# johanDDC/R-TuckER

Measured on AMD Instinct MI355X. Metric: 1-vs-N triples scored/sec, higher is better.
Workload: dtype f32

## Files before the change

r-tucker_amd/csrc/rtk_score_cg_kernel.h:

```cpp
#pragma once
#include "rtk_common.h"
#include "rtk_pack.h"
#include <type_traits>

namespace rtk_cg {

#ifdef RTK_CG_STAMPS
static __device__ unsigned long long g_cg_tl[256 * 2 * 64];
#define RTK_CG_TL(role, code)                                                                                   \
    do {                                                                                                        \
        if (tl_on && tl_n < 64) {                                                                               \
            g_cg_tl[(blockIdx.x * 2 + (role)) * 64 + tl_n] =                                                    \
                ((unsigned long long)(code) << 56) | (__builtin_amdgcn_s_memtime() & 0x00ffffffffffffffull);    \
            ++tl_n;                                                                                             \
        }                                                                                                       \
    } while (0)
#define RTK_CG_TLR(role, code)                                                                                  \
    do {                                                                                                        \
        if (tl_on && tl_n < 64) {                                                                               \
            g_cg_tl[(blockIdx.x * 2 + (role)) * 64 + tl_n] =                                                    \
                ((unsigned long long)(code) << 56) | (__builtin_amdgcn_s_memrealtime() & 0x00ffffffffffffffull); \
            ++tl_n;                                                                                             \
        }                                                                                                       \
    } while (0)
#else
#define RTK_CG_TL(role, code) do { (void)tl_on; (void)tl_n; } while (0)
#define RTK_CG_TLR(role, code) do { (void)tl_on; (void)tl_n; } while (0)
#endif

constexpr int NG = 5;
constexpr int EX_BYTES = 4 * 4 * 64 * 16;
constexpr int MISC_BYTES = 1024;

template <int KS>
__host__ __device__ constexpr int tile_bytes() { return RTK_PACK_HDR + 2 * KS * 1024; }

template <int KS>
inline size_t lds_bytes(int) { return MISC_BYTES + 2 * (size_t)tile_bytes<KS>() + 4 * (size_t)EX_BYTES; }

__host__ __device__ constexpr int s_begin(int KS, int w) { return (KS * w + 3) / 4; }
__host__ __device__ constexpr int s_end(int KS, int w) { return (KS * (w + 1) + 3) / 4; }

struct Geo {
    int B, N, c, U, n_mt;
    int gq, gr;
    int64_t ld_out;
    __device__ __forceinline__ int first_group(int u) const {
        if (U <= 32768) return gq * u + (int)((unsigned)(gr * u) / (unsigned)U);
        return (int)((((int64_t)gq * U + gr) * u) / U);
    }
    __device__ __forceinline__ void set(int u, int &gb, int &n_g) const {
        gb = first_group(u);
        n_g = first_group(u + 1) - gb;
    }
};

typedef float f32x2 __attribute__((ext_vector_type(2)));
typedef _Float16 f16x2 __attribute__((ext_vector_type(2)));

__device__ __forceinline__ void split8(const f32x4 a, const f32x4 b, float up, f16x8 &hi, f16x8 &lo) {
    const f32x2 u2 = {up, up};
    f32x2 y[4] = {{a[0], a[1]}, {a[2], a[3]}, {b[0], b[1]}, {b[2], b[3]}};
    union { f16x2 h2[4]; f16x8 h8; unsigned u[4]; } H, Lo;
#pragma unroll
    for (int j = 0; j < 4; ++j) {
        y[j] = y[j] * u2;
        H.h2[j] = __builtin_convertvector(y[j], f16x2);
        unsigned l;
        asm("v_fma_mixlo_f16 %0, %1, 1.0, -%2 op_sel_hi:[0,0,1]" : "=v"(l) : "v"(y[j][0]), "v"(H.u[j]));
        asm("v_fma_mixhi_f16 %0, %1, 1.0, -%2 op_sel:[0,0,1] op_sel_hi:[0,0,1]" : "+v"(l) : "v"(y[j][1]), "v"(H.u[j]));
        Lo.u[j] = l;
    }
    hi = H.h8;
    lo = Lo.h8;
}

template <int KS, int K0, int K1>
__device__ __forceinline__ void load_fragments_raw(__amdgpu_buffer_rsrc_t rs, unsigned n_bytes, int row, int c, int h, f32x4 *rw) {
    const unsigned base = (unsigned)(row * c + 8 * h) * 4u;
    const int k_last = 16 * (KS - 1) + 8 * h;
    const unsigned base_a = (k_last + 4 <= c) ? base : n_bytes, base_b = (k_last + 8 <= c) ? base : n_bytes;
#pragma unroll
    for (int ks = K0; ks < K1; ++ks) {
        const bool last = ks + 1 == KS;
        rw[2 * (ks - K0)] = __builtin_bit_cast(f32x4, __builtin_amdgcn_raw_buffer_load_b128(rs, last ? base_a : base, 64 * ks, 0));
        rw[2 * (ks - K0) + 1] = __builtin_bit_cast(f32x4, __builtin_amdgcn_raw_buffer_load_b128(rs, last ? base_b : base, 64 * ks + 16, 0));
    }
}

template <int NP>
__device__ __forceinline__ float row_absmax(const f32x4 *rw) {
    float mx = 0.f;
#pragma unroll
    for (int i = 0; i + 1 < NP; i += 2) {
#pragma unroll
        for (int q = 0; q < 4; ++q)
            asm("v_max3_f32 %0, |%1|, |%2|, %0" : "+v"(mx) : "v"(rw[i][q]), "v"(rw[i + 1][q]));
    }
    return fmaxf(mx, __shfl_xor(mx, 32));
}

struct LdsMap {
    unsigned char *hdr;
    float *uso5;
    float *pmax;
    unsigned char *stg0, *stg1;
    unsigned char *exo;
    unsigned char *exp5;
    template <int KS>
    __device__ __forceinline__ void init(unsigned char *lds) {
        hdr = lds;
        uso5 = reinterpret_cast<float *>(lds + 384);
        pmax = reinterpret_cast<float *>(lds + 512);
        stg0 = lds + MISC_BYTES;
        stg1 = stg0 + tile_bytes<KS>();
        exo = stg1 + tile_bytes<KS>();
        exp5 = exo + 2 * EX_BYTES;
    }
};

struct MOut {
    float *out;
    int64_t ld_out;
    int B, nts;
    unsigned voff;
};

template <int KS, int W4, int SIGMOID, bool EXTRA>
__device__ __forceinline__ void m_sweep(const LdsMap &L, int cnt, int lane, const f16x8 (&BF)[2 * KS],
                                        const f16x8 *SF, float us_o, const MOut &mo, bool tl_on, int &tl_n) {
#ifndef RTK_CG_PF
#define RTK_CG_PF 3
#endif
    constexpr int PF = KS < RTK_CG_PF ? KS : RTK_CG_PF;
    constexpr int S0 = s_begin(KS, W4), S1 = s_end(KS, W4), NS = EXTRA ? S1 - S0 : 0;
    constexpr int NGAP = 3 * KS + 3 * NS;
    constexpr int PW0 = !EXTRA ? (1 << 20) : (NS > 0 ? 3 * S1 + 3 * NS + 2 : 32);
    constexpr int GEND = EXTRA ? (PW0 + 4 > 36 ? PW0 + 4 : 36) : 32;
    constexpr bool MSIG = SIGMOID == 2;
    const int h = lane >> 5;
    const float kfac = MSIG ? us_o * -1.4426950408889634f : us_o;
    float ee = 0.f;
    f32x16 accA, accB, accS;
#pragma unroll
    for (int e = 0; e < 16; ++e) accB[e] = 0.f, accS[e] = 0.f;
    const f32x16 zero = {0.f, 0.f, 0.f, 0.f, 0.f, 0.f, 0.f, 0.f, 0.f, 0.f, 0.f, 0.f, 0.f, 0.f, 0.f, 0.f};

    auto iteration = [&](auto par_c, auto chain_c, auto pieces_c, int i, f32x16 &accC, f32x16 &accP) {
        constexpr int PAR = decltype(par_c)::value;
        constexpr bool chain = decltype(chain_c)::value, pieces = decltype(pieces_c)::value;
        constexpr bool direct = !chain && pieces;
        f32x4 *exw = reinterpret_cast<f32x4 *>(L.exo + (PAR ^ 1) * EX_BYTES + W4 * 4096);
        f32x4 *exs = reinterpret_cast<f32x4 *>(L.exp5 + PAR * EX_BYTES + W4 * 4096);
        const float *rfp = reinterpret_cast<const float *>(L.hdr + ((i + 2) % 3) * 128) + 4 * h;
        f32x4 rfq[2];
        auto gap = [&](int g) {
            if (EXTRA && g >= PW0 && g < PW0 + 4) {
                if (chain) {
                    const int q = g - PW0;
                    exs[q * 64 + lane] = f32x4{accS[4 * q], accS[4 * q + 1], accS[4 * q + 2], accS[4 * q + 3]};
                }
                return;
            }
            const int p = g - ((EXTRA && g >= PW0 + 4) ? 4 : 0);
            if (p >= 32 || !pieces) return;
            const int e = p >> 1, eg = e >> 2;
            if ((p & 7) == 1 && eg < 3) rfq[(eg + 1) & 1] = *reinterpret_cast<const f32x4 *>(rfp + 8 * (eg + 1));
            if (MSIG) {
                if (!(p & 1)) {
                    ee = __builtin_amdgcn_exp2f(accP[e] * rfq[eg & 1][e & 3] * kfac);
                } else {
                    accP[e] = __builtin_amdgcn_rcpf(1.0f + ee);
                    if ((e & 3) == 3 && !direct) exw[eg * 64 + lane] = f32x4{accP[e - 3], accP[e - 2], accP[e - 1], accP[e]};
                }
            } else if ((p & 7) == 0) {
                f32x4 z;
#pragma unroll
                for (int q = 0; q < 4; ++q) z[q] = accP[4 * eg + q] * rfq[eg & 1][q] * kfac;
                if (direct) {
#pragma unroll
                    for (int q = 0; q < 4; ++q) accP[4 * eg + q] = (SIGMOID == 1) ? rtk_sigmoid(z[q]) : z[q];
                } else {
                    exw[eg * 64 + lane] = z;
                }
            }
        };
        if (pieces) rfq[0] = *reinterpret_cast<const f32x4 *>(rfp);
        if constexpr (chain) {
            const unsigned char *tile = PAR ? L.stg1 : L.stg0;
            const f16x8 *lh = reinterpret_cast<const f16x8 *>(tile + RTK_PACK_HDR);
            const f16x8 *ll = lh + KS * 64;
            f16x8 fa[PF], fl[PF];
#pragma unroll
            for (int p = 0; p < PF; ++p) {
                fa[p] = lh[p * 64 + lane];
                fl[p] = ll[p * 64 + lane];
            }
            int g = 0;
#pragma unroll
            for (int ks = 0; ks < KS; ++ks) {
                const f16x8 ah = fa[ks % PF], al = fl[ks % PF];
                if (ks + PF < KS) {
                    fa[ks % PF] = lh[(ks + PF) * 64 + lane];
                    fl[ks % PF] = ll[(ks + PF) * 64 + lane];
                }
                const bool sh = EXTRA && ks >= S0 && ks < S1;
                __builtin_amdgcn_sched_barrier(0);
                accC = __builtin_amdgcn_mfma_f32_32x32x16_f16(ah, BF[2 * ks], ks == 0 ? zero : accC, 0, 0, 0);
                __builtin_amdgcn_sched_barrier(0);
                gap(g++);
                __builtin_amdgcn_sched_barrier(0);
                if (sh) {
                    accS = __builtin_amdgcn_mfma_f32_32x32x16_f16(ah, SF[2 * (ks - S0)], ks == S0 ? zero : accS, 0, 0, 0);
                    __builtin_amdgcn_sched_barrier(0);
                    gap(g++);
                    __builtin_amdgcn_sched_barrier(0);
                }
                accC = __builtin_amdgcn_mfma_f32_32x32x16_f16(ah, BF[2 * ks + 1], accC, 0, 0, 0);
                __builtin_amdgcn_sched_barrier(0);
                gap(g++);
                __builtin_amdgcn_sched_barrier(0);
                if (sh) {
                    accS = __builtin_amdgcn_mfma_f32_32x32x16_f16(ah, SF[2 * (ks - S0) + 1], accS, 0, 0, 0);
                    __builtin_amdgcn_sched_barrier(0);
                    gap(g++);
                    __builtin_amdgcn_sched_barrier(0);
                }
                accC = __builtin_amdgcn_mfma_f32_32x32x16_f16(al, BF[2 * ks], accC, 0, 0, 0);
                __builtin_amdgcn_sched_barrier(0);
                gap(g++);
                __builtin_amdgcn_sched_barrier(0);
                if (sh) {
                    accS = __builtin_amdgcn_mfma_f32_32x32x16_f16(al, SF[2 * (ks - S0)], accS, 0, 0, 0);
                    __builtin_amdgcn_sched_barrier(0);
                    gap(g++);
                    __builtin_amdgcn_sched_barrier(0);
                }
            }
#pragma unroll
            for (int gg = NGAP; gg < GEND; ++gg) gap(gg);
        } else if constexpr (pieces) {
#pragma unroll
            for (int gg = 0; gg < 32; ++gg) gap(gg + ((EXTRA && gg >= PW0) ? 4 : 0));
            const __amdgpu_buffer_rsrc_t rs = __builtin_amdgcn_make_buffer_rsrc(
                mo.out + (int64_t)(i - 1) * 32 * mo.ld_out, 0, (unsigned)(min(32, mo.B - (i - 1) * 32) * mo.ld_out * 4), 0x00020000);
            const unsigned ld4 = (unsigned)(mo.ld_out * 4);
            auto put = [&](auto aux_c) {
                unsigned off = mo.voff;
#pragma unroll
                for (int e = 0; e < 16; ++e) {
                    const float pe = accP[e];
                    __builtin_amdgcn_raw_buffer_store_b32(__builtin_bit_cast(unsigned, pe), rs, off, 0, decltype(aux_c)::value);
                    off += ((e & 3) == 3) ? 5u * ld4 : ld4;
                }
            };
            if (mo.nts) put(std::integral_constant<int, 2>{});
            else put(std::integral_constant<int, 0>{});
        }
        RTK_CG_TL(0, 6);
        __syncthreads();
        RTK_CG_TL(0, 5);
    };
    using P0 = std::integral_constant<int, 0>;
    using P1 = std::integral_constant<int, 1>;
    using T = std::true_type;
    using F = std::false_type;
    iteration(P0{}, T{}, F{}, 0, accA, accB);
    int i = 1;
    for (; i + 1 < cnt; i += 2) {
        iteration(P1{}, T{}, T{}, i, accB, accA);
        iteration(P0{}, T{}, T{}, i + 1, accA, accB);
    }
    if (i < cnt) {
        iteration(P1{}, T{}, T{}, i, accB, accA);
        iteration(P0{}, F{}, T{}, i + 1, accA, accB);
    } else {
        iteration(P1{}, F{}, T{}, i, accB, accA);
    }
}

template <int KS, int W4, int SIGMOID>
__device__ __forceinline__ void m_role(const Geo &geo, const float *__restrict__ O, float *__restrict__ out,
                                       const LdsMap &L, int lane, int nts) {
    constexpr int S0 = s_begin(KS, W4), S1 = s_end(KS, W4), NS = S1 - S0;
    const int r = lane & 31, h = lane >> 5, c = geo.c;
    const bool tl_on = W4 == 0 && lane == 0;
    int tl_n = 0;
    RTK_CG_TLR(0, 12);
    for (int u = blockIdx.x; u < geo.U; u += gridDim.x) {
        int gb, n_g;
        geo.set(u, gb, n_g);
        RTK_CG_TL(0, 1);
        const bool own = W4 < n_g;
        constexpr int NSX = NS > 0 ? NS : 1;
        f16x8 BF[2 * KS], SF[2 * NSX];
        float us_o = 0.f;
        {
            const int64_t row0 = (int64_t)gb * 32;
            const int valid_rows = (int)max((int64_t)0, min((int64_t)n_g * 32, (int64_t)geo.N - row0));
            const __amdgpu_buffer_rsrc_t rs = __builtin_amdgcn_make_buffer_rsrc(
                const_cast<float *>(O + row0 * c), 0, (unsigned)valid_rows * (unsigned)c * 4u, 0x00020000);
            const unsigned n_bytes = (unsigned)valid_rows * (unsigned)c * 4u;
            if (NS > 0) load_fragments_raw<KS, S0, S1>(rs, n_bytes, 4 * 32 + r, c, h, reinterpret_cast<f32x4 *>(SF));
            load_fragments_raw<KS, 0, KS>(rs, n_bytes, W4 * 32 + r, c, h, reinterpret_cast<f32x4 *>(BF));
            const float pm = NS > 0 ? row_absmax<2 * NSX>(reinterpret_cast<const f32x4 *>(SF)) : 0.f;
            if (h == 0) L.pmax[W4 * 32 + r] = pm;
            RTK_CG_TL(0, 2);
            __syncthreads();
            if (n_g == NG) {
                const float m5 = fmaxf(fmaxf(L.pmax[r], L.pmax[32 + r]), fmaxf(L.pmax[64 + r], L.pmax[96 + r]));
                const int sh5 = rtk_pack_shift(m5);
                const float up5 = ldexpf(1.0f, sh5);
#pragma unroll
                for (int ks = 0; ks < NS; ++ks)
                    split8(__builtin_bit_cast(f32x4, SF[2 * ks]), __builtin_bit_cast(f32x4, SF[2 * ks + 1]), up5, SF[2 * ks], SF[2 * ks + 1]);
                if (W4 == 0 && h == 0) L.uso5[r] = ldexpf(1.0f, -sh5);
            }
            RTK_CG_TL(0, 7);
            if (own) {
                const int sh = rtk_pack_shift(row_absmax<2 * KS>(reinterpret_cast<const f32x4 *>(BF)));
                const float up = ldexpf(1.0f, sh);
#pragma unroll
                for (int ks = 0; ks < KS; ++ks)
                    split8(__builtin_bit_cast(f32x4, BF[2 * ks]), __builtin_bit_cast(f32x4, BF[2 * ks + 1]), up, BF[2 * ks], BF[2 * ks + 1]);
                us_o = ldexpf(1.0f, -sh);
            }
        }
        RTK_CG_TL(0, 3);
        __syncthreads();
        RTK_CG_TL(0, 4);
        MOut mo;
        mo.out = out; mo.ld_out = geo.ld_out; mo.B = geo.B; mo.nts = nts;
        {
            const int j = (gb + W4) * 32 + r;
            mo.voff = (own && j < geo.N) ? (unsigned)(4 * h * geo.ld_out * 4) + (unsigned)j * 4u : 0x80000000u;
        }
        if (!own) {
            for (int i = 0; i < geo.n_mt + 1; ++i) __syncthreads();
        } else if (n_g == NG) {
            m_sweep<KS, W4, SIGMOID, true>(L, geo.n_mt, lane, BF, SF, us_o, mo, tl_on, tl_n);
        } else {
            m_sweep<KS, W4, SIGMOID, false>(L, geo.n_mt, lane, BF, SF, us_o, mo, tl_on, tl_n);
        }
    }
    RTK_CG_TLR(0, 13);
}

template <int AUX>
__device__ __forceinline__ void store_five(const float (&p5)[4], __amdgpu_buffer_rsrc_t rs, unsigned voff, unsigned ld4) {
    unsigned off = voff;
#pragma unroll
    for (int q = 0; q < 4; ++q) {
        __builtin_amdgcn_raw_buffer_store_b32(__builtin_bit_cast(unsigned, p5[q]), rs, off, 0, AUX);
        off += ld4;
    }
}

template <int KS>
__device__ __forceinline__ void h_prologue(const unsigned char *__restrict__ q_packed, const LdsMap &L, int t) {
    constexpr int TILE_BYTES = tile_bytes<KS>();
    constexpr int CHUNKS = TILE_BYTES / 16;
    constexpr int NLD = (CHUNKS + 255) / 256;
    const int ht = t & 255;
    u32x4 sreg[NLD];
    const u32x4 *src = reinterpret_cast<const u32x4 *>(q_packed);
#pragma unroll
    for (int i = 0; i < NLD; ++i) {
        const int ch = i * 256 + ht;
        if (i + 1 < NLD || ch < CHUNKS) sreg[i] = src[ch];
    }
    u32x4 *dst = reinterpret_cast<u32x4 *>(L.stg0);
#pragma unroll
    for (int i = 0; i < NLD; ++i) {
        const int ch = i * 256 + ht;
        if (i + 1 < NLD || ch < CHUNKS) dst[ch] = sreg[i];
    }
    if (ht < RTK_PACK_HDR / 16) reinterpret_cast<u32x4 *>(L.hdr)[ht] = sreg[0];
}

template <int KS, int SIGMOID, int SW>
__device__ __forceinline__ void s_role(const Geo &geo, const unsigned char *__restrict__ q_packed,
                                       float *__restrict__ out, const LdsMap &L, int lane, int t, int nts, int tune) {
    constexpr int NU = (20 - SW + 2) / 3;
    const int r = lane & 31, h = lane >> 5, N = geo.N, B = geo.B;
    const int64_t ld_out = geo.ld_out;
    const unsigned ld4 = (unsigned)(ld_out * 4);
    const int cnt = geo.n_mt;
    const bool tl_on = SW == 0 && lane == 0;
    int tl_n = 0;
    for (int u = blockIdx.x; u < geo.U; u += gridDim.x) {
        int gb, n_g;
        geo.set(u, gb, n_g);
        RTK_CG_TL(1, 1);
        h_prologue<KS>(q_packed, L, t);
        RTK_CG_TL(1, 2);
        const bool five = n_g == NG;
        __syncthreads();
        __syncthreads();
        RTK_CG_TL(1, 4);
        const unsigned row4h = (unsigned)(4 * h * ld_out * 4);
        unsigned colb[5];
#pragma unroll
        for (int g = 0; g < 5; ++g) {
            const int j = (gb + g) * 32 + r;
            colb[g] = (g < n_g && j < N) ? row4h + (unsigned)j * 4u : 0x80000000u;
        }
        float k5 = five ? L.uso5[r] : 0.f;
        if (SIGMOID == 2) k5 *= -1.4426950408889634f;
        for (int i = 0; i < cnt + 1; ++i) {
            const bool st_own = i >= 2, st5 = five && i >= 1 && i <= cnt;
            f32x4 z[NU], p1[2], p2[2], p3[2], rf[2];
            const f32x4 *ex = reinterpret_cast<const f32x4 *>(L.exo + (i & 1) * EX_BYTES) + lane;
            const f32x4 *pr = reinterpret_cast<const f32x4 *>(L.exp5 + ((i - 1) & 1) * EX_BYTES) + lane;
            const unsigned char *rp = L.hdr + ((i + 2) % 3) * 128 + 4 * h * 4;
#pragma unroll
            for (int k = 0; k < NU; ++k) {
                constexpr int dummy = 0;
                (void)dummy;
                const int uu = SW + 3 * k;
                if (uu < 16) {
                    if (st_own) z[k] = ex[(uu >> 2) * 256 + (uu & 3) * 64];
                } else if (st5) {
                    const int b = uu - 16, kk = k - (NU - (SW == 2 ? 1 : (SW == 1 ? 2 : 1)));
                    z[k] = pr[b * 64];
                    p1[kk] = pr[256 + b * 64];
                    p2[kk] = pr[512 + b * 64];
                    p3[kk] = pr[768 + b * 64];
                    rf[kk] = *reinterpret_cast<const f32x4 *>(rp + b * 32);
                }
            }
            RTK_CG_TL(1, 11);
            const __amdgpu_buffer_rsrc_t rs_own = __builtin_amdgcn_make_buffer_rsrc(
                out + (int64_t)(i - 2) * 32 * ld_out, 0, (unsigned)(min(32, B - (i - 2) * 32) * ld_out * 4), 0x00020000);
            const __amdgpu_buffer_rsrc_t rs5 = __builtin_amdgcn_make_buffer_rsrc(
                out + (int64_t)(i - 1) * 32 * ld_out, 0, (unsigned)(min(32, B - (i - 1) * 32) * ld_out * 4), 0x00020000);
#pragma unroll
            for (int k = 0; k < NU; ++k) {
                const int uu = SW + 3 * k;
                float p[4];
                if (uu < 16) {
                    if (!st_own) continue;
#pragma unroll
                    for (int q = 0; q < 4; ++q) p[q] = (SIGMOID == 1) ? rtk_sigmoid(z[k][q]) : z[k][q];
                    const unsigned voff = colb[uu >> 2] + (unsigned)(uu & 3) * 8u * ld4;
                    if (tune & 16) asm volatile("" ::"v"(p[0]), "v"(p[1]), "v"(p[2]), "v"(p[3]));
                    else if (nts) store_five<2>(p, rs_own, voff, ld4);
                    else store_five<0>(p, rs_own, voff, ld4);
                } else {
                    if (!st5) continue;
                    const int b = uu - 16, kk = k - (NU - (SW == 2 ? 1 : (SW == 1 ? 2 : 1)));
#pragma unroll
                    for (int q = 0; q < 4; ++q) {
                        const float zz = (((z[k][q] + p1[kk][q]) + p2[kk][q]) + p3[kk][q]) * rf[kk][q] * k5;
                        p[q] = SIGMOID == 2 ? __builtin_amdgcn_rcpf(1.0f + __builtin_amdgcn_exp2f(zz))
                                            : (SIGMOID == 1 ? rtk_sigmoid(zz) : zz);
                    }
                    const unsigned voff = colb[4] + (unsigned)b * 8u * ld4;
                    if (tune & 16) asm volatile("" ::"v"(p[0]), "v"(p[1]), "v"(p[2]), "v"(p[3]));
                    else if (nts) store_five<2>(p, rs5, voff, ld4);
                    else store_five<0>(p, rs5, voff, ld4);
                }
            }
            RTK_CG_TL(1, 6);
            __syncthreads();
            RTK_CG_TL(1, 5);
        }
    }
}

template <int KS>
__device__ __forceinline__ void l_role(const Geo &geo, const unsigned char *__restrict__ q_packed,
                                       const LdsMap &L, int lane, int t, int tune) {
    constexpr int TILE_BYTES = tile_bytes<KS>();
    constexpr int CHUNKS = TILE_BYTES / 16;
    constexpr int NLD = (CHUNKS + 63) / 64;
    const int cnt = geo.n_mt;
    u32x4 sreg[NLD];
    const __amdgpu_buffer_rsrc_t rsq = __builtin_amdgcn_make_buffer_rsrc(
        const_cast<unsigned char *>(q_packed), 0, (unsigned)(cnt * TILE_BYTES), 0x00020000);
    auto stage_load = [&](int mt) {
#pragma unroll
        for (int i = 0; i < NLD; ++i)
            sreg[i] = __builtin_amdgcn_raw_buffer_load_b128(rsq, (unsigned)lane * 16u, mt * TILE_BYTES + i * 1024, 0);
    };
    auto stage_store = [&](int mt) {
        u32x4 *dst = reinterpret_cast<u32x4 *>((mt & 1) ? L.stg1 : L.stg0);
#pragma unroll
        for (int i = 0; i < NLD; ++i) {
            const int ch = i * 64 + lane;
            if (i + 1 < NLD || ch < CHUNKS) dst[ch] = sreg[i];
        }
        if (lane < RTK_PACK_HDR / 16) reinterpret_cast<u32x4 *>(L.hdr + (mt % 3) * 128)[lane] = sreg[0];
    };
    for (int u = blockIdx.x; u < geo.U; u += gridDim.x) {
        int gb, n_g;
        geo.set(u, gb, n_g);
        h_prologue<KS>(q_packed, L, t);
        if (cnt > 1 && !(tune & 32)) stage_load(1);
        __syncthreads();
        __syncthreads();
        for (int i = 0; i < cnt + 1; ++i) {
            if (i + 1 < cnt && !(tune & 32)) stage_store(i + 1);
            if (i + 2 < cnt && !(tune & 32)) stage_load(i + 2);
            __syncthreads();
        }
    }
}

template <int KS, int SIGMOID>
__global__ __launch_bounds__(512, 2) void score_cg_kernel(
    const unsigned char *__restrict__ q_packed, int B, const float *__restrict__ O, int N, int c,
    float *__restrict__ out, int64_t ld_out, int U, int gq, int gr, int nts, int tune) {
    extern __shared__ __attribute__((aligned(16))) unsigned char lds[];
    LdsMap L;
    L.init<KS>(lds);
    const int t = threadIdx.x, lane = t & 63, wave = t >> 6;
    Geo geo;
    geo.B = B; geo.N = N; geo.c = c; geo.U = U; geo.gq = gq; geo.gr = gr; geo.n_mt = (B + 31) / 32; geo.ld_out = ld_out;
    const int uwave = __builtin_amdgcn_readfirstlane(wave);
    {
        const int pr = __builtin_amdgcn_readfirstlane(uwave >= 4 ? (tune & 3) : ((tune >> 2) & 3));
        if (pr == 1) __builtin_amdgcn_s_setprio(1);
        else if (pr == 2) __builtin_amdgcn_s_setprio(2);
        else if (pr == 3) __builtin_amdgcn_s_setprio(3);
    }
#ifdef RTK_CG_STAMPS
    if ((uwave == 0 || uwave == 4) && lane == 0)
        g_cg_tl[(blockIdx.x * 2 + (uwave >> 2)) * 64 + 63] = __builtin_amdgcn_s_memtime();
#endif
    if (uwave == 0) m_role<KS, 0, SIGMOID>(geo, O, out, L, lane, __builtin_amdgcn_readfirstlane(nts));
    else if (uwave == 1) m_role<KS, 1, SIGMOID>(geo, O, out, L, lane, __builtin_amdgcn_readfirstlane(nts));
    else if (uwave == 2) m_role<KS, 2, SIGMOID>(geo, O, out, L, lane, __builtin_amdgcn_readfirstlane(nts));
    else if (uwave == 3) m_role<KS, 3, SIGMOID>(geo, O, out, L, lane, __builtin_amdgcn_readfirstlane(nts));
    else if (uwave == 4) s_role<KS, SIGMOID, 0>(geo, q_packed, out, L, lane, t, __builtin_amdgcn_readfirstlane(nts), __builtin_amdgcn_readfirstlane(tune));
    else if (uwave == 5) s_role<KS, SIGMOID, 1>(geo, q_packed, out, L, lane, t, __builtin_amdgcn_readfirstlane(nts), __builtin_amdgcn_readfirstlane(tune));
    else if (uwave == 6) s_role<KS, SIGMOID, 2>(geo, q_packed, out, L, lane, t, __builtin_amdgcn_readfirstlane(nts), __builtin_amdgcn_readfirstlane(tune));
    else l_role<KS>(geo, q_packed, L, lane, t, __builtin_amdgcn_readfirstlane(tune));
}

}
```

Baseline: 11.42 million.

## Pipeline fp32-to-split-fp16 fragment conversion into the first tile's MFMA chain

The prologue used to split every owned and shared k-step fragment into hi/lo fp16 before the first barrier. Now it converts only the first k-step. The remaining conversions are done in three stages (scale, round/lo, hi) and slotted into the gap slots between MFMAs of tile 0's chain, so they overlap matrix work instead of stalling it. The row absmax is computed before the barrier, and the sweep tail loop is restructured. This raises register pressure and adds scheduling complexity, and the extra-group path now runs m_sweep even for non-owning waves.

New measurement: 11.37 million. Within noise of the previous version (-0.4%).

```diff
diff --git a/r-tucker_amd/csrc/rtk_score_cg_kernel.h b/r-tucker_amd/csrc/rtk_score_cg_kernel.h
--- a/r-tucker_amd/csrc/rtk_score_cg_kernel.h
+++ b/r-tucker_amd/csrc/rtk_score_cg_kernel.h
@@ -58,21 +58,35 @@
 typedef float f32x2 __attribute__((ext_vector_type(2)));
 typedef _Float16 f16x2 __attribute__((ext_vector_type(2)));
 
+struct Split {
+    f32x2 y[4];
+    unsigned h[4], l[4];
+    __device__ __forceinline__ void scale(const f32x4 a, const f32x4 b, f32x2 up2) {
+        const f32x2 r[4] = {{a[0], a[1]}, {a[2], a[3]}, {b[0], b[1]}, {b[2], b[3]}};
+#pragma unroll
+        for (int j = 0; j < 4; ++j) asm volatile("v_pk_mul_f32 %0, %1, %2" : "=v"(y[j]) : "v"(r[j]), "v"(up2));
+    }
+    __device__ __forceinline__ void round_lo() {
+#pragma unroll
+        for (int j = 0; j < 4; ++j) asm volatile("v_cvt_pk_f16_f32 %0, %1, %2" : "=v"(h[j]) : "v"(y[j][0]), "v"(y[j][1]));
+#pragma unroll
+        for (int j = 0; j < 4; ++j)
+            asm volatile("v_fma_mixlo_f16 %0, %1, 1.0, -%2 op_sel_hi:[0,0,1]" : "=v"(l[j]) : "v"(y[j][0]), "v"(h[j]));
+    }
+    __device__ __forceinline__ void hi_out(f16x8 &hi, f16x8 &lo) {
+#pragma unroll
+        for (int j = 0; j < 4; ++j)
+            asm volatile("v_fma_mixhi_f16 %0, %1, 1.0, -%2 op_sel:[0,0,1] op_sel_hi:[0,0,1]" : "+v"(l[j]) : "v"(y[j][1]), "v"(h[j]));
+        hi = __builtin_bit_cast(f16x8, u32x4{h[0], h[1], h[2], h[3]});
+        lo = __builtin_bit_cast(f16x8, u32x4{l[0], l[1], l[2], l[3]});
+    }
+};
+
 __device__ __forceinline__ void split8(const f32x4 a, const f32x4 b, float up, f16x8 &hi, f16x8 &lo) {
-    const f32x2 u2 = {up, up};
-    f32x2 y[4] = {{a[0], a[1]}, {a[2], a[3]}, {b[0], b[1]}, {b[2], b[3]}};
-    union { f16x2 h2[4]; f16x8 h8; unsigned u[4]; } H, Lo;
-#pragma unroll
-    for (int j = 0; j < 4; ++j) {
-        y[j] = y[j] * u2;
-        H.h2[j] = __builtin_convertvector(y[j], f16x2);
-        unsigned l;
-        asm("v_fma_mixlo_f16 %0, %1, 1.0, -%2 op_sel_hi:[0,0,1]" : "=v"(l) : "v"(y[j][0]), "v"(H.u[j]));
-        asm("v_fma_mixhi_f16 %0, %1, 1.0, -%2 op_sel:[0,0,1] op_sel_hi:[0,0,1]" : "+v"(l) : "v"(y[j][1]), "v"(H.u[j]));
-        Lo.u[j] = l;
-    }
-    hi = H.h8;
-    lo = Lo.h8;
+    Split sp;
+    sp.scale(a, b, f32x2{up, up});
+    sp.round_lo();
+    sp.hi_out(hi, lo);
 }
 
 template <int KS, int K0, int K1>
@@ -126,9 +140,15 @@
     unsigned voff;
 };
 
-template <int KS, int W4, int SIGMOID, bool EXTRA>
-__device__ __forceinline__ void m_sweep(const LdsMap &L, int cnt, int lane, const f16x8 (&BF)[2 * KS],
-                                        const f16x8 *SF, float us_o, const MOut &mo, bool tl_on, int &tl_n) {
+#ifdef RTK_CG_SERIAL_PROLOGUE
+constexpr bool PIPELINED = false;
+#else
+constexpr bool PIPELINED = true;
+#endif
+
+template <int KS, int W4, int SIGMOID, bool EXTRA, int NSX>
+__device__ __forceinline__ void m_sweep(const LdsMap &L, int cnt, int lane, f16x8 (&BF)[2 * KS], f16x8 (&SF)[2 * NSX],
+                                        float up, float up5, float us_o, const MOut &mo, bool tl_on, int &tl_n) {
 #ifndef RTK_CG_PF
 #define RTK_CG_PF 3
 #endif
@@ -140,16 +160,19 @@
     constexpr bool MSIG = SIGMOID == 2;
     const int h = lane >> 5;
     const float kfac = MSIG ? us_o * -1.4426950408889634f : us_o;
+    const f32x2 up2 = {up, up}, up52 = {up5, up5};
     float ee = 0.f;
     f32x16 accA, accB, accS;
 #pragma unroll
     for (int e = 0; e < 16; ++e) accB[e] = 0.f, accS[e] = 0.f;
     const f32x16 zero = {0.f, 0.f, 0.f, 0.f, 0.f, 0.f, 0.f, 0.f, 0.f, 0.f, 0.f, 0.f, 0.f, 0.f, 0.f, 0.f};
 
-    auto iteration = [&](auto par_c, auto chain_c, auto pieces_c, int i, f32x16 &accC, f32x16 &accP) {
+    auto iteration = [&](auto par_c, auto chain_c, auto pieces_c, auto convert_c, int i, f32x16 &accC, f32x16 &accP) {
         constexpr int PAR = decltype(par_c)::value;
         constexpr bool chain = decltype(chain_c)::value, pieces = decltype(pieces_c)::value;
+        constexpr bool convert = decltype(convert_c)::value && PIPELINED;
         constexpr bool direct = !chain && pieces;
+        static_assert(!convert || (chain && !pieces), "the conversion rides in tile 0's chain");
         f32x4 *exw = reinterpret_cast<f32x4 *>(L.exo + (PAR ^ 1) * EX_BYTES + W4 * 4096);
         f32x4 *exs = reinterpret_cast<f32x4 *>(L.exp5 + PAR * EX_BYTES + W4 * 4096);
         const float *rfp = reinterpret_cast<const float *>(L.hdr + ((i + 2) % 3) * 128) + 4 * h;
@@ -185,6 +208,19 @@
                 }
             }
         };
+        Split cs[2];
+        auto stage = [&](auto which_c, int kk, int st) {
+            constexpr int X = decltype(which_c)::value;
+            f16x8 &fh = X ? SF[2 * kk] : BF[2 * kk], &fl = X ? SF[2 * kk + 1] : BF[2 * kk + 1];
+            if (st == 0) cs[X].scale(__builtin_bit_cast(f32x4, fh), __builtin_bit_cast(f32x4, fl), X ? up52 : up2);
+            else if (st == 1) cs[X].round_lo();
+            else cs[X].hi_out(fh, fl);
+        };
+        auto convert_ahead = [&](int ks, int slot, int nslots) {
+            const bool own_next = ks + 1 < KS, sh_next = EXTRA && ks + 1 >= S0 && ks + 1 < S1;
+            if (own_next && slot < 3) stage(std::integral_constant<int, 0>{}, ks + 1, slot);
+            if (sh_next && slot >= nslots - 3) stage(std::integral_constant<int, 1>{}, ks + 1 - S0, slot - (nslots - 3));
+        };
         if (pieces) rfq[0] = *reinterpret_cast<const f32x4 *>(rfp);
         if constexpr (chain) {
             const unsigned char *tile = PAR ? L.stg1 : L.stg0;
@@ -205,38 +241,46 @@
                     fl[ks % PF] = ll[(ks + PF) * 64 + lane];
                 }
                 const bool sh = EXTRA && ks >= S0 && ks < S1;
+                int slot = 0;
+                auto fill = [&] {
+                    gap(g++);
+                    if constexpr (convert) convert_ahead(ks, slot, sh ? 6 : 3);
+                    ++slot;
+                };
+                if (convert && ks == 0) RTK_CG_TL(0, 14);
                 __builtin_amdgcn_sched_barrier(0);
                 accC = __builtin_amdgcn_mfma_f32_32x32x16_f16(ah, BF[2 * ks], ks == 0 ? zero : accC, 0, 0, 0);
                 __builtin_amdgcn_sched_barrier(0);
-                gap(g++);
+                fill();
                 __builtin_amdgcn_sched_barrier(0);
                 if (sh) {
                     accS = __builtin_amdgcn_mfma_f32_32x32x16_f16(ah, SF[2 * (ks - S0)], ks == S0 ? zero : accS, 0, 0, 0);
                     __builtin_amdgcn_sched_barrier(0);
-                    gap(g++);
+                    fill();
                     __builtin_amdgcn_sched_barrier(0);
                 }
                 accC = __builtin_amdgcn_mfma_f32_32x32x16_f16(ah, BF[2 * ks + 1], accC, 0, 0, 0);
                 __builtin_amdgcn_sched_barrier(0);
-                gap(g++);
+                fill();
                 __builtin_amdgcn_sched_barrier(0);
                 if (sh) {
                     accS = __builtin_amdgcn_mfma_f32_32x32x16_f16(ah, SF[2 * (ks - S0) + 1], accS, 0, 0, 0);
                     __builtin_amdgcn_sched_barrier(0);
-                    gap(g++);
+                    fill();
                     __builtin_amdgcn_sched_barrier(0);
                 }
                 accC = __builtin_amdgcn_mfma_f32_32x32x16_f16(al, BF[2 * ks], accC, 0, 0, 0);
                 __builtin_amdgcn_sched_barrier(0);
-                gap(g++);
+                fill();
                 __builtin_amdgcn_sched_barrier(0);
                 if (sh) {
                     accS = __builtin_amdgcn_mfma_f32_32x32x16_f16(al, SF[2 * (ks - S0)], accS, 0, 0, 0);
                     __builtin_amdgcn_sched_barrier(0);
-                    gap(g++);
+                    fill();
                     __builtin_amdgcn_sched_barrier(0);
                 }
             }
+            if (convert) RTK_CG_TL(0, 15);
 #pragma unroll
             for (int gg = NGAP; gg < GEND; ++gg) gap(gg);
         } else if constexpr (pieces) {
@@ -265,18 +309,18 @@
     using P1 = std::integral_constant<int, 1>;
     using T = std::true_type;
     using F = std::false_type;
-    iteration(P0{}, T{}, F{}, 0, accA, accB);
+    iteration(P0{}, T{}, F{}, T{}, 0, accA, accB);
     int i = 1;
-    for (; i + 1 < cnt; i += 2) {
-        iteration(P1{}, T{}, T{}, i, accB, accA);
-        iteration(P0{}, T{}, T{}, i + 1, accA, accB);
-    }
-    if (i < cnt) {
-        iteration(P1{}, T{}, T{}, i, accB, accA);
-        iteration(P0{}, F{}, T{}, i + 1, accA, accB);
-    } else {
-        iteration(P1{}, F{}, T{}, i, accB, accA);
-    }
+    for (; i < cnt; i += 2) {
+        iteration(P1{}, T{}, T{}, F{}, i, accB, accA);
+        if (i + 1 == cnt) {
+            accA = accB;
+            ++i;
+            break;
+        }
+        iteration(P0{}, T{}, T{}, F{}, i + 1, accA, accB);
+    }
+    iteration(P1{}, F{}, T{}, F{}, i, accB, accA);
 }
 
 template <int KS, int W4, int SIGMOID>
@@ -292,56 +336,66 @@
         geo.set(u, gb, n_g);
         RTK_CG_TL(0, 1);
         const bool own = W4 < n_g;
-        constexpr int NSX = NS > 0 ? NS : 1;
-        f16x8 BF[2 * KS], SF[2 * NSX];
-        float us_o = 0.f;
-        {
-            const int64_t row0 = (int64_t)gb * 32;
-            const int valid_rows = (int)max((int64_t)0, min((int64_t)n_g * 32, (int64_t)geo.N - row0));
-            const __amdgpu_buffer_rsrc_t rs = __builtin_amdgcn_make_buffer_rsrc(
-                const_cast<float *>(O + row0 * c), 0, (unsigned)valid_rows * (unsigned)c * 4u, 0x00020000);
-            const unsigned n_bytes = (unsigned)valid_rows * (unsigned)c * 4u;
-            if (NS > 0) load_fragments_raw<KS, S0, S1>(rs, n_bytes, 4 * 32 + r, c, h, reinterpret_cast<f32x4 *>(SF));
-            load_fragments_raw<KS, 0, KS>(rs, n_bytes, W4 * 32 + r, c, h, reinterpret_cast<f32x4 *>(BF));
-            const float pm = NS > 0 ? row_absmax<2 * NSX>(reinterpret_cast<const f32x4 *>(SF)) : 0.f;
-            if (h == 0) L.pmax[W4 * 32 + r] = pm;
-            RTK_CG_TL(0, 2);
+        auto pass = [&](auto extra_c) {
+            constexpr bool EXTRA = decltype(extra_c)::value;
+            if constexpr (EXTRA) asm volatile("; pass: set with a fifth group" ::: "memory");
+            else asm volatile("; pass: set of up to four groups" ::: "memory");
+            constexpr int NSX = NS > 0 ? NS : 1;
+            constexpr bool shared = EXTRA && NS > 0;
+            f16x8 BF[2 * KS], SF[2 * NSX];
+            constexpr int KS_FRONT = PIPELINED ? 1 : KS, NS_FRONT = !shared ? 0 : (PIPELINED ? (S0 == 0 ? 1 : 0) : NS);
+            float us_o = 0.f, up = 0.f, up5 = 0.f;
+            {
+                const int64_t row0 = (int64_t)gb * 32;
+                const int valid_rows = (int)max((int64_t)0, min((int64_t)n_g * 32, (int64_t)geo.N - row0));
+                const __amdgpu_buffer_rsrc_t rs = __builtin_amdgcn_make_buffer_rsrc(
+                    const_cast<float *>(O + row0 * c), 0, (unsigned)valid_rows * (unsigned)c * 4u, 0x00020000);
+                const unsigned n_bytes = (unsigned)valid_rows * (unsigned)c * 4u;
+                if (shared) load_fragments_raw<KS, S0, S1>(rs, n_bytes, 4 * 32 + r, c, h, reinterpret_cast<f32x4 *>(SF));
+                load_fragments_raw<KS, 0, KS>(rs, n_bytes, W4 * 32 + r, c, h, reinterpret_cast<f32x4 *>(BF));
+                if (EXTRA) {
+                    const float pm = shared ? row_absmax<2 * NSX>(reinterpret_cast<const f32x4 *>(SF)) : 0.f;
+                    if (h == 0) L.pmax[W4 * 32 + r] = pm;
+                }
+                const float om = PIPELINED ? row_absmax<2 * KS>(reinterpret_cast<const f32x4 *>(BF)) : 0.f;
+                RTK_CG_TL(0, 2);
+                __syncthreads();
+                if (EXTRA) {
+                    const float m5 = fmaxf(fmaxf(L.pmax[r], L.pmax[32 + r]), fmaxf(L.pmax[64 + r], L.pmax[96 + r]));
+                    const int sh5 = rtk_pack_shift(m5);
+                    up5 = ldexpf(1.0f, sh5);
+#pragma unroll
+                    for (int ks = 0; ks < NS_FRONT; ++ks)
+                        split8(__builtin_bit_cast(f32x4, SF[2 * ks]), __builtin_bit_cast(f32x4, SF[2 * ks + 1]), up5, SF[2 * ks], SF[2 * ks + 1]);
+                    if (W4 == 0 && h == 0) L.uso5[r] = ldexpf(1.0f, -sh5);
+                }
+                RTK_CG_TL(0, 7);
+                if (own) {
+                    const int sh = rtk_pack_shift(PIPELINED ? om : row_absmax<2 * KS>(reinterpret_cast<const f32x4 *>(BF)));
+                    up = ldexpf(1.0f, sh);
+#pragma unroll
+                    for (int ks = 0; ks < KS_FRONT; ++ks)
+                        split8(__builtin_bit_cast(f32x4, BF[2 * ks]), __builtin_bit_cast(f32x4, BF[2 * ks + 1]), up, BF[2 * ks], BF[2 * ks + 1]);
+                    us_o = ldexpf(1.0f, -sh);
+                }
+            }
+            RTK_CG_TL(0, 3);
             __syncthreads();
-            if (n_g == NG) {
-                const float m5 = fmaxf(fmaxf(L.pmax[r], L.pmax[32 + r]), fmaxf(L.pmax[64 + r], L.pmax[96 + r]));
-                const int sh5 = rtk_pack_shift(m5);
-                const float up5 = ldexpf(1.0f, sh5);
-#pragma unroll
-                for (int ks = 0; ks < NS; ++ks)
-                    split8(__builtin_bit_cast(f32x4, SF[2 * ks]), __builtin_bit_cast(f32x4, SF[2 * ks + 1]), up5, SF[2 * ks], SF[2 * ks + 1]);
-                if (W4 == 0 && h == 0) L.uso5[r] = ldexpf(1.0f, -sh5);
-            }
-            RTK_CG_TL(0, 7);
-            if (own) {
-                const int sh = rtk_pack_shift(row_absmax<2 * KS>(reinterpret_cast<const f32x4 *>(BF)));
-                const float up = ldexpf(1.0f, sh);
-#pragma unroll
-                for (int ks = 0; ks < KS; ++ks)
-                    split8(__builtin_bit_cast(f32x4, BF[2 * ks]), __builtin_bit_cast(f32x4, BF[2 * ks + 1]), up, BF[2 * ks], BF[2 * ks + 1]);
-                us_o = ldexpf(1.0f, -sh);
-            }
-        }
-        RTK_CG_TL(0, 3);
-        __syncthreads();
-        RTK_CG_TL(0, 4);
-        MOut mo;
-        mo.out = out; mo.ld_out = geo.ld_out; mo.B = geo.B; mo.nts = nts;
-        {
-            const int j = (gb + W4) * 32 + r;
-            mo.voff = (own && j < geo.N) ? (unsigned)(4 * h * geo.ld_out * 4) + (unsigned)j * 4u : 0x80000000u;
-        }
-        if (!own) {
-            for (int i = 0; i < geo.n_mt + 1; ++i) __syncthreads();
-        } else if (n_g == NG) {
-            m_sweep<KS, W4, SIGMOID, true>(L, geo.n_mt, lane, BF, SF, us_o, mo, tl_on, tl_n);
-        } else {
-            m_sweep<KS, W4, SIGMOID, false>(L, geo.n_mt, lane, BF, SF, us_o, mo, tl_on, tl_n);
-        }
+            RTK_CG_TL(0, 4);
+            MOut mo;
+            mo.out = out; mo.ld_out = geo.ld_out; mo.B = geo.B; mo.nts = nts;
+            {
+                const int j = (gb + W4) * 32 + r;
+                mo.voff = (own && j < geo.N) ? (unsigned)(4 * h * geo.ld_out * 4) + (unsigned)j * 4u : 0x80000000u;
+            }
+            if (EXTRA || own) {
+                m_sweep<KS, W4, SIGMOID, EXTRA, NSX>(L, geo.n_mt, lane, BF, SF, up, up5, us_o, mo, tl_on, tl_n);
+            } else {
+                for (int i = 0; i < geo.n_mt + 1; ++i) __syncthreads();
+            }
+        };
+        if (n_g == NG) pass(std::true_type{});
+        else pass(std::false_type{});
     }
     RTK_CG_TLR(0, 13);
 }
```
